# LikeLy-Journey/SegmenTron

Hardware: AMD Instinct MI355X
Metric: images/sec fwd+bwd DeepLabv3+_xception65 @1025x2049 (higher is better)
Workload: dtype bf16; 1 GPU; DeepLabv3+_xception65 train step (fwd + CE loss + bwd + SGD) @1025x2049, batch 2/GPU (BASELINE.json configs[2]); global_batch=2, bn=BN, parallelism=dp1, full_size=True

## Files before the change

segmentron_amd/csrc/optim.hip:

```cpp
#include "common.h"

namespace seg {

constexpr int SGD_TENSORS = 48;
constexpr int SGD_BLOCKS = 320;
constexpr int SGD_CHUNK = 16384;
constexpr int SGD_THREADS = 256;

struct SgdArgs {
  float* p[SGD_TENSORS];
  const float* g[SGD_TENSORS];
  float* m[SGD_TENSORS];
  int n[SGD_TENSORS];
  unsigned char group[SGD_TENSORS];
  unsigned char blk_tensor[SGD_BLOCKS];
  int blk_chunk[SGD_BLOCKS];
  const float* lr;
  const float* wd;
  float momentum;
  int first;
};

__global__ __launch_bounds__(SGD_THREADS) void sgd_multi_tensor_kernel(const SgdArgs a) {
  const int t = a.blk_tensor[blockIdx.x];
  const long base = (long)a.blk_chunk[blockIdx.x] * SGD_CHUNK;
  const int n = a.n[t];
  float* __restrict__ p = a.p[t];
  const float* __restrict__ g = a.g[t];
  float* __restrict__ m = a.m[t];
  const float lr = a.lr[a.group[t]], wd = a.wd[a.group[t]];
  const float mom = a.momentum;
  const bool vec = (n % 4) == 0;
  if (vec) {
    for (long i = base + threadIdx.x * 4; i < min((long)n, base + SGD_CHUNK); i += SGD_THREADS * 4) {
      float4 pv = *reinterpret_cast<float4*>(p + i);
      const float4 gv = *reinterpret_cast<const float4*>(g + i);
      float4 mv = make_float4(0.f, 0.f, 0.f, 0.f);
      if (!a.first) mv = *reinterpret_cast<float4*>(m + i);
      float pe[4] = {pv.x, pv.y, pv.z, pv.w}, me[4] = {mv.x, mv.y, mv.z, mv.w};
      const float ge[4] = {gv.x, gv.y, gv.z, gv.w};
#pragma unroll
      for (int k = 0; k < 4; ++k) {
        const float d = fmaf(wd, pe[k], ge[k]);
        me[k] = a.first ? d : fmaf(mom, me[k], d);
        pe[k] = fmaf(-lr, me[k], pe[k]);
      }
      *reinterpret_cast<float4*>(m + i) = make_float4(me[0], me[1], me[2], me[3]);
      *reinterpret_cast<float4*>(p + i) = make_float4(pe[0], pe[1], pe[2], pe[3]);
    }
  } else {
    for (long i = base + threadIdx.x; i < min((long)n, base + SGD_CHUNK); i += SGD_THREADS) {
      const float d = fmaf(wd, p[i], g[i]);
      const float mv = a.first ? d : fmaf(mom, m[i], d);
      m[i] = mv;
      p[i] = fmaf(-lr, mv, p[i]);
    }
  }
}

}

extern "C" int seg_sgd_multi_tensor(int ntensors, const void* const* params,
                                    const void* const* grads, const void* const* bufs,
                                    const long* numel, const int* group, const float* lr_dev,
                                    const float* wd_dev, float momentum, int first, void* stream) {
  using namespace seg;
  SEG_REQUIRE(ntensors >= 0 && lr_dev && wd_dev, "sgd_multi_tensor: bad arguments");
  SgdArgs a;
  a.lr = lr_dev; a.wd = wd_dev; a.momentum = momentum; a.first = first ? 1 : 0;
  int nt = 0, nb = 0;
  auto flush = [&]() -> int {
    if (nb == 0) { nt = 0; return 0; }
    hipLaunchKernelGGL(sgd_multi_tensor_kernel, dim3(nb), dim3(SGD_THREADS), 0,
                       (hipStream_t)stream, a);
    nt = nb = 0;
    return check_launch("sgd_multi_tensor");
  };
  for (int i = 0; i < ntensors; ++i) {
    SEG_REQUIRE(params[i] && grads[i] && bufs[i], "sgd_multi_tensor: null tensor %d", i);
    SEG_REQUIRE(numel[i] >= 0 && numel[i] < (1L << 31), "sgd_multi_tensor: tensor %d too large", i);
    SEG_REQUIRE(group[i] >= 0 && group[i] < 256, "sgd_multi_tensor: bad group %d", group[i]);
    const int chunks = (int)((numel[i] + SGD_CHUNK - 1) / SGD_CHUNK);
    int c = 0;
    while (c < chunks) {
      if (nt == SGD_TENSORS || nb == SGD_BLOCKS) {
        const int rc = flush();
        if (rc) return rc;
      }
      a.p[nt] = (float*)params[i]; a.g[nt] = (const float*)grads[i]; a.m[nt] = (float*)bufs[i];
      a.n[nt] = (int)numel[i]; a.group[nt] = (unsigned char)group[i];
      while (c < chunks && nb < SGD_BLOCKS) {
        a.blk_tensor[nb] = (unsigned char)nt;
        a.blk_chunk[nb] = c;
        ++nb; ++c;
      }
      ++nt;
    }
  }
  return flush();
}


namespace seg {

constexpr int PK_JOBS = 32, PK_BLOCKS = 480, PK_TILE = 64, PK_THREADS = 256;
constexpr int PK_SPAN = 4;

struct PackArgs {
  const float* src[PK_JOBS];
  void* dst[PK_JOBS];
  int O[PK_JOBS], C[PK_JOBS];
  unsigned char transpose[PK_JOBS];
  unsigned char blk_job[PK_BLOCKS];
  int blk_tile[PK_BLOCKS];
  int dtype;
};

template <typename T>
__global__ __launch_bounds__(PK_THREADS) void pack_multi_kernel(const PackArgs a) {
  __shared__ float tile[PK_TILE][PK_TILE + 1];
  const int j = a.blk_job[blockIdx.x];
  const int O = a.O[j], C = a.C[j];
  const int tc = (C + PK_TILE - 1) / PK_TILE, ntiles = ((O + PK_TILE - 1) / PK_TILE) * tc;
  const float* __restrict__ src = a.src[j];
  T* __restrict__ dst = reinterpret_cast<T*>(a.dst[j]);
  const int tx = threadIdx.x & 63, ty = threadIdx.x >> 6;
  const bool tr = a.transpose[j] != 0;
  for (int t = a.blk_tile[blockIdx.x]; t < min(ntiles, a.blk_tile[blockIdx.x] + PK_SPAN); ++t) {
    const int o0 = (t / tc) * PK_TILE, c0 = (t % tc) * PK_TILE;
    if (!tr) {
      for (int r = ty; r < PK_TILE; r += 4) {
        const int o = o0 + r, c = c0 + tx;
        if (o < O && c < C) Vec<T>::store1(dst + (long)o * C + c, src[(long)o * C + c]);
      }
      continue;
    }
    __syncthreads();
    for (int r = ty; r < PK_TILE; r += 4) {
      const int o = o0 + r, c = c0 + tx;
      tile[r][tx] = (o < O && c < C) ? src[(long)o * C + c] : 0.f;
    }
    __syncthreads();
    for (int r = ty; r < PK_TILE; r += 4) {
      const int c = c0 + r, o = o0 + tx;
      if (c < C && o < O) Vec<T>::store1(dst + (long)c * O + o, tile[tx][r]);
    }
  }
}

}

extern "C" int seg_pack_multi(int dtype, int njobs, const void* const* srcs, const void* const* dsts,
                              const int* O, const int* C, const int* transpose, void* stream) {
  using namespace seg;
  SEG_REQUIRE(dtype == DT_F32 || dtype == DT_BF16, "pack_multi: bad dtype %d", dtype);
  PackArgs a;
  a.dtype = dtype;
  int nj = 0, nb = 0;
  auto flush = [&]() -> int {
    if (nb == 0) { nj = 0; return 0; }
    if (dtype == DT_BF16)
      hipLaunchKernelGGL((pack_multi_kernel<bf16_t>), dim3(nb), dim3(PK_THREADS), 0,
                         (hipStream_t)stream, a);
    else
      hipLaunchKernelGGL((pack_multi_kernel<float>), dim3(nb), dim3(PK_THREADS), 0,
                         (hipStream_t)stream, a);
    nj = nb = 0;
    return check_launch("pack_multi");
  };
  for (int i = 0; i < njobs; ++i) {
    SEG_REQUIRE(srcs[i] && dsts[i] && O[i] >= 1 && C[i] >= 1, "pack_multi: bad job %d", i);
    const long to = (O[i] + PK_TILE - 1) / PK_TILE, tc = (C[i] + PK_TILE - 1) / PK_TILE;
    SEG_REQUIRE(to * tc < (1L << 30), "pack_multi: job %d too large", i);
    long t = 0;
    while (t < to * tc) {
      if (nj == PK_JOBS || nb == PK_BLOCKS) {
        const int rc = flush();
        if (rc) return rc;
      }
      a.src[nj] = (const float*)srcs[i]; a.dst[nj] = const_cast<void*>(dsts[i]);
      a.O[nj] = O[i]; a.C[nj] = C[i]; a.transpose[nj] = transpose[i] ? 1 : 0;
      while (t < to * tc && nb < PK_BLOCKS) {
        a.blk_job[nb] = (unsigned char)nj;
        a.blk_tile[nb] = (int)t;
        ++nb; t += PK_SPAN;
      }
      ++nj;
    }
  }
  return flush();
}
```

Baseline: 91.37 images/sec.

## Rework multi-tensor SGD and weight-pack kernels with binary-search block planning

Moves the SGD and pack launch planning into a shared header. Each block now finds its tensor by binary search over per-tensor first-block offsets, which lets one launch cover many more tensors and cuts launch count. SGD is templated on the first step, unrolled with nontemporal loads and stores, and uses smaller chunks. Pack merges a plain copy and a transposed copy of the same source into one job and uses vectorized 8-wide loads and stores. The costs are extra per-block search work and more complex alignment-dependent code paths.

```diff
diff --git a/segmentron_amd/csrc/optim.hip b/segmentron_amd/csrc/optim.hip
--- a/segmentron_amd/csrc/optim.hip
+++ b/segmentron_amd/csrc/optim.hip
@@ -1,57 +1,69 @@
 #include "common.h"
+#include "optim_plan.h"
 
 namespace seg {
 
-constexpr int SGD_TENSORS = 48;
-constexpr int SGD_BLOCKS = 320;
-constexpr int SGD_CHUNK = 16384;
-constexpr int SGD_THREADS = 256;
-
-struct SgdArgs {
-  float* p[SGD_TENSORS];
-  const float* g[SGD_TENSORS];
-  float* m[SGD_TENSORS];
-  int n[SGD_TENSORS];
-  unsigned char group[SGD_TENSORS];
-  unsigned char blk_tensor[SGD_BLOCKS];
-  int blk_chunk[SGD_BLOCKS];
-  const float* lr;
-  const float* wd;
-  float momentum;
-  int first;
-};
-
+__device__ __forceinline__ bool aligned16(const void* p) { return ((uintptr_t)p & 15) == 0; }
+
+__device__ __forceinline__ float4 ldg_nt(const float* p) {
+  const f32x4 v = __builtin_nontemporal_load(reinterpret_cast<const f32x4*>(p));
+  return make_float4(v.x, v.y, v.z, v.w);
+}
+__device__ __forceinline__ void stg_nt(float* p, const float4& v) {
+  const f32x4 t = {v.x, v.y, v.z, v.w};
+  __builtin_nontemporal_store(t, reinterpret_cast<f32x4*>(p));
+}
+
+template <bool FIRST>
 __global__ __launch_bounds__(SGD_THREADS) void sgd_multi_tensor_kernel(const SgdArgs a) {
-  const int t = a.blk_tensor[blockIdx.x];
-  const long base = (long)a.blk_chunk[blockIdx.x] * SGD_CHUNK;
+  const int t = plan_find(a.first_blk, a.nt, (int)blockIdx.x);
+  const long base = (long)((int)blockIdx.x - a.first_blk[t]) * SGD_CHUNK;
   const int n = a.n[t];
   float* __restrict__ p = a.p[t];
   const float* __restrict__ g = a.g[t];
   float* __restrict__ m = a.m[t];
   const float lr = a.lr[a.group[t]], wd = a.wd[a.group[t]];
   const float mom = a.momentum;
-  const bool vec = (n % 4) == 0;
+  const long end = min((long)n, base + SGD_CHUNK);
+  const bool vec = (n % 4) == 0 && aligned16(p) && aligned16(g) && aligned16(m);
   if (vec) {
-    for (long i = base + threadIdx.x * 4; i < min((long)n, base + SGD_CHUNK); i += SGD_THREADS * 4) {
-      float4 pv = *reinterpret_cast<float4*>(p + i);
-      const float4 gv = *reinterpret_cast<const float4*>(g + i);
-      float4 mv = make_float4(0.f, 0.f, 0.f, 0.f);
-      if (!a.first) mv = *reinterpret_cast<float4*>(m + i);
-      float pe[4] = {pv.x, pv.y, pv.z, pv.w}, me[4] = {mv.x, mv.y, mv.z, mv.w};
-      const float ge[4] = {gv.x, gv.y, gv.z, gv.w};
-#pragma unroll
-      for (int k = 0; k < 4; ++k) {
-        const float d = fmaf(wd, pe[k], ge[k]);
-        me[k] = a.first ? d : fmaf(mom, me[k], d);
-        pe[k] = fmaf(-lr, me[k], pe[k]);
-      }
-      *reinterpret_cast<float4*>(m + i) = make_float4(me[0], me[1], me[2], me[3]);
-      *reinterpret_cast<float4*>(p + i) = make_float4(pe[0], pe[1], pe[2], pe[3]);
+    for (long b = base; b < end; b += SGD_THREADS * 4 * SGD_UNROLL) {
+      long idx[SGD_UNROLL];
+      bool ok[SGD_UNROLL];
+      float4 pv[SGD_UNROLL], gv[SGD_UNROLL], mv[SGD_UNROLL];
+#pragma unroll
+      for (int u = 0; u < SGD_UNROLL; ++u) {
+        const long i = b + (long)(u * SGD_THREADS + (int)threadIdx.x) * 4;
+        ok[u] = i < end;
+        idx[u] = ok[u] ? i : end - 4;
+      }
+#pragma unroll
+      for (int u = 0; u < SGD_UNROLL; ++u) {
+        pv[u] = *reinterpret_cast<const float4*>(p + idx[u]);
+        gv[u] = ldg_nt(g + idx[u]);
+        mv[u] = FIRST ? make_float4(0.f, 0.f, 0.f, 0.f) : ldg_nt(m + idx[u]);
+      }
+#pragma unroll
+      for (int u = 0; u < SGD_UNROLL; ++u) {
+        float pe[4] = {pv[u].x, pv[u].y, pv[u].z, pv[u].w};
+        float me[4] = {mv[u].x, mv[u].y, mv[u].z, mv[u].w};
+        const float ge[4] = {gv[u].x, gv[u].y, gv[u].z, gv[u].w};
+#pragma unroll
+        for (int k = 0; k < 4; ++k) {
+          const float d = fmaf(wd, pe[k], ge[k]);
+          me[k] = FIRST ? d : fmaf(mom, me[k], d);
+          pe[k] = fmaf(-lr, me[k], pe[k]);
+        }
+        if (ok[u]) {
+          stg_nt(m + idx[u], make_float4(me[0], me[1], me[2], me[3]));
+          *reinterpret_cast<float4*>(p + idx[u]) = make_float4(pe[0], pe[1], pe[2], pe[3]);
+        }
+      }
     }
   } else {
-    for (long i = base + threadIdx.x; i < min((long)n, base + SGD_CHUNK); i += SGD_THREADS) {
+    for (long i = base + threadIdx.x; i < end; i += SGD_THREADS) {
       const float d = fmaf(wd, p[i], g[i]);
-      const float mv = a.first ? d : fmaf(mom, m[i], d);
+      const float mv = FIRST ? d : fmaf(mom, m[i], d);
       m[i] = mv;
       p[i] = fmaf(-lr, mv, p[i]);
     }
@@ -66,84 +78,106 @@
                                     const float* wd_dev, float momentum, int first, void* stream) {
   using namespace seg;
   SEG_REQUIRE(ntensors >= 0 && lr_dev && wd_dev, "sgd_multi_tensor: bad arguments");
+  for (int i = 0; i < ntensors; ++i) {
+    SEG_REQUIRE(numel[i] >= 0 && numel[i] < (1L << 31), "sgd_multi_tensor: tensor %d too large", i);
+    SEG_REQUIRE(numel[i] == 0 || (params[i] && grads[i] && bufs[i]),
+                "sgd_multi_tensor: null tensor %d", i);
+    SEG_REQUIRE(group[i] >= 0 && group[i] < 256, "sgd_multi_tensor: bad group %d", group[i]);
+  }
   SgdArgs a;
-  a.lr = lr_dev; a.wd = wd_dev; a.momentum = momentum; a.first = first ? 1 : 0;
-  int nt = 0, nb = 0;
-  auto flush = [&]() -> int {
-    if (nb == 0) { nt = 0; return 0; }
-    hipLaunchKernelGGL(sgd_multi_tensor_kernel, dim3(nb), dim3(SGD_THREADS), 0,
-                       (hipStream_t)stream, a);
-    nt = nb = 0;
+  a.lr = lr_dev; a.wd = wd_dev; a.momentum = momentum;
+  return sgd_plan(ntensors, params, grads, bufs, numel, group, a, [&](const SgdArgs& l, int nb) {
+    if (first)
+      hipLaunchKernelGGL(sgd_multi_tensor_kernel<true>, dim3(nb), dim3(SGD_THREADS), 0,
+                         (hipStream_t)stream, l);
+    else
+      hipLaunchKernelGGL(sgd_multi_tensor_kernel<false>, dim3(nb), dim3(SGD_THREADS), 0,
+                         (hipStream_t)stream, l);
     return check_launch("sgd_multi_tensor");
-  };
-  for (int i = 0; i < ntensors; ++i) {
-    SEG_REQUIRE(params[i] && grads[i] && bufs[i], "sgd_multi_tensor: null tensor %d", i);
-    SEG_REQUIRE(numel[i] >= 0 && numel[i] < (1L << 31), "sgd_multi_tensor: tensor %d too large", i);
-    SEG_REQUIRE(group[i] >= 0 && group[i] < 256, "sgd_multi_tensor: bad group %d", group[i]);
-    const int chunks = (int)((numel[i] + SGD_CHUNK - 1) / SGD_CHUNK);
-    int c = 0;
-    while (c < chunks) {
-      if (nt == SGD_TENSORS || nb == SGD_BLOCKS) {
-        const int rc = flush();
-        if (rc) return rc;
-      }
-      a.p[nt] = (float*)params[i]; a.g[nt] = (const float*)grads[i]; a.m[nt] = (float*)bufs[i];
-      a.n[nt] = (int)numel[i]; a.group[nt] = (unsigned char)group[i];
-      while (c < chunks && nb < SGD_BLOCKS) {
-        a.blk_tensor[nb] = (unsigned char)nt;
-        a.blk_chunk[nb] = c;
-        ++nb; ++c;
-      }
-      ++nt;
-    }
-  }
-  return flush();
+  });
 }
 
 
 namespace seg {
-
-constexpr int PK_JOBS = 32, PK_BLOCKS = 480, PK_TILE = 64, PK_THREADS = 256;
-constexpr int PK_SPAN = 4;
-
-struct PackArgs {
-  const float* src[PK_JOBS];
-  void* dst[PK_JOBS];
-  int O[PK_JOBS], C[PK_JOBS];
-  unsigned char transpose[PK_JOBS];
-  unsigned char blk_job[PK_BLOCKS];
-  int blk_tile[PK_BLOCKS];
-  int dtype;
-};
 
 template <typename T>
 __global__ __launch_bounds__(PK_THREADS) void pack_multi_kernel(const PackArgs a) {
+  constexpr int VEC = Vec<T>::N;
   __shared__ float tile[PK_TILE][PK_TILE + 1];
-  const int j = a.blk_job[blockIdx.x];
+  const int j = plan_find(a.first_blk, a.nj, (int)blockIdx.x);
+  const int t = (int)blockIdx.x - a.first_blk[j];
   const int O = a.O[j], C = a.C[j];
-  const int tc = (C + PK_TILE - 1) / PK_TILE, ntiles = ((O + PK_TILE - 1) / PK_TILE) * tc;
+  const int tc = (C + PK_TILE - 1) / PK_TILE;
+  const int o0 = (t / tc) * PK_TILE, c0 = (t % tc) * PK_TILE;
   const float* __restrict__ src = a.src[j];
   T* __restrict__ dst = reinterpret_cast<T*>(a.dst[j]);
-  const int tx = threadIdx.x & 63, ty = threadIdx.x >> 6;
-  const bool tr = a.transpose[j] != 0;
-  for (int t = a.blk_tile[blockIdx.x]; t < min(ntiles, a.blk_tile[blockIdx.x] + PK_SPAN); ++t) {
-    const int o0 = (t / tc) * PK_TILE, c0 = (t % tc) * PK_TILE;
-    if (!tr) {
-      for (int r = ty; r < PK_TILE; r += 4) {
-        const int o = o0 + r, c = c0 + tx;
-        if (o < O && c < C) Vec<T>::store1(dst + (long)o * C + c, src[(long)o * C + c]);
-      }
-      continue;
-    }
-    __syncthreads();
+  T* __restrict__ dst_t = reinterpret_cast<T*>(a.dst_t[j]);
+  const int tid = threadIdx.x;
+  if ((C % 8) == 0 && aligned16(src)) {
+    const int c8 = tid & 7, r = tid >> 3;
+    const int c = c0 + c8 * 8;
+    const bool cok = c < C;
+    const int cl = cok ? c : C - 8;
+    const bool wide_dst = dst != nullptr && aligned16(dst);
+    float4 w[2][2];
+#pragma unroll
+    for (int i = 0; i < 2; ++i) {
+      const int o = min(o0 + r + 32 * i, O - 1);
+      w[i][0] = *reinterpret_cast<const float4*>(src + (long)o * C + cl);
+      w[i][1] = *reinterpret_cast<const float4*>(src + (long)o * C + cl + 4);
+    }
+#pragma unroll
+    for (int i = 0; i < 2; ++i) {
+      const int ro = r + 32 * i, o = o0 + ro;
+      const float f[8] = {w[i][0].x, w[i][0].y, w[i][0].z, w[i][0].w,
+                          w[i][1].x, w[i][1].y, w[i][1].z, w[i][1].w};
+      if (dst != nullptr && o < O && cok) {
+        T* d = dst + (long)o * C + c;
+        if (wide_dst) {
+#pragma unroll
+          for (int k = 0; k < 8; k += VEC) Vec<T>::store(d + k, f + k);
+        } else {
+#pragma unroll
+          for (int k = 0; k < 8; ++k) Vec<T>::store1(d + k, f[k]);
+        }
+      }
+      if (dst_t != nullptr) {
+#pragma unroll
+        for (int k = 0; k < 8; ++k) tile[ro][c8 * 8 + k] = f[k];
+      }
+    }
+  } else {
+    const int tx = tid & 63, ty = tid >> 6;
     for (int r = ty; r < PK_TILE; r += 4) {
       const int o = o0 + r, c = c0 + tx;
-      tile[r][tx] = (o < O && c < C) ? src[(long)o * C + c] : 0.f;
-    }
-    __syncthreads();
+      const bool ok = o < O && c < C;
+      const float v = ok ? src[(long)o * C + c] : 0.f;
+      if (ok && dst != nullptr) Vec<T>::store1(dst + (long)o * C + c, v);
+      if (dst_t != nullptr) tile[r][tx] = v;
+    }
+  }
+  if (dst_t == nullptr) return;
+  __syncthreads();
+  if ((O % 8) == 0 && aligned16(dst_t)) {
+#pragma unroll
+    for (int i = 0; i < 2; ++i) {
+      const int idx = tid + PK_THREADS * i;
+      const int og = idx & 7, cl = idx >> 3;
+      const int o = o0 + og * 8, c = c0 + cl;
+      if (c < C && o < O) {
+        float f[8];
+#pragma unroll
+        for (int k = 0; k < 8; ++k) f[k] = tile[og * 8 + k][cl];
+        T* d = dst_t + (long)c * O + o;
+#pragma unroll
+        for (int k = 0; k < 8; k += VEC) Vec<T>::store(d + k, f + k);
+      }
+    }
+  } else {
+    const int tx = tid & 63, ty = tid >> 6;
     for (int r = ty; r < PK_TILE; r += 4) {
       const int c = c0 + r, o = o0 + tx;
-      if (c < C && o < O) Vec<T>::store1(dst + (long)c * O + o, tile[tx][r]);
+      if (c < C && o < O) Vec<T>::store1(dst_t + (long)c * O + o, tile[tx][r]);
     }
   }
 }
@@ -154,39 +188,18 @@
                               const int* O, const int* C, const int* transpose, void* stream) {
   using namespace seg;
   SEG_REQUIRE(dtype == DT_F32 || dtype == DT_BF16, "pack_multi: bad dtype %d", dtype);
+  for (int i = 0; i < njobs; ++i) {
+    SEG_REQUIRE(srcs[i] && dsts[i] && O[i] >= 1 && C[i] >= 1, "pack_multi: bad job %d", i);
+    SEG_REQUIRE(pack_tiles(O[i], C[i]) < (1L << 30), "pack_multi: job %d too large", i);
+  }
   PackArgs a;
-  a.dtype = dtype;
-  int nj = 0, nb = 0;
-  auto flush = [&]() -> int {
-    if (nb == 0) { nj = 0; return 0; }
+  return pack_plan(njobs, srcs, dsts, O, C, transpose, a, [&](const PackArgs& l, int nb) {
     if (dtype == DT_BF16)
       hipLaunchKernelGGL((pack_multi_kernel<bf16_t>), dim3(nb), dim3(PK_THREADS), 0,
-                         (hipStream_t)stream, a);
+                         (hipStream_t)stream, l);
     else
       hipLaunchKernelGGL((pack_multi_kernel<float>), dim3(nb), dim3(PK_THREADS), 0,
-                         (hipStream_t)stream, a);
-    nj = nb = 0;
+                         (hipStream_t)stream, l);
     return check_launch("pack_multi");
-  };
-  for (int i = 0; i < njobs; ++i) {
-    SEG_REQUIRE(srcs[i] && dsts[i] && O[i] >= 1 && C[i] >= 1, "pack_multi: bad job %d", i);
-    const long to = (O[i] + PK_TILE - 1) / PK_TILE, tc = (C[i] + PK_TILE - 1) / PK_TILE;
-    SEG_REQUIRE(to * tc < (1L << 30), "pack_multi: job %d too large", i);
-    long t = 0;
-    while (t < to * tc) {
-      if (nj == PK_JOBS || nb == PK_BLOCKS) {
-        const int rc = flush();
-        if (rc) return rc;
-      }
-      a.src[nj] = (const float*)srcs[i]; a.dst[nj] = const_cast<void*>(dsts[i]);
-      a.O[nj] = O[i]; a.C[nj] = C[i]; a.transpose[nj] = transpose[i] ? 1 : 0;
-      while (t < to * tc && nb < PK_BLOCKS) {
-        a.blk_job[nb] = (unsigned char)nj;
-        a.blk_tile[nb] = (int)t;
-        ++nb; t += PK_SPAN;
-      }
-      ++nj;
-    }
-  }
-  return flush();
-}
+  });
+}
diff --git a/segmentron_amd/csrc/optim_plan.h b/segmentron_amd/csrc/optim_plan.h
--- /dev/null
+++ b/segmentron_amd/csrc/optim_plan.h
@@ -0,0 +1,125 @@
+#pragma once
+#include <stdint.h>
+#include <vector>
+
+#if defined(__HIPCC__)
+#define SEG_PLAN_HD __host__ __device__ __forceinline__
+#else
+#define SEG_PLAN_HD inline
+#endif
+
+namespace seg {
+
+constexpr int PLAN_ARG_BYTES = 4096;
+
+SEG_PLAN_HD int plan_find(const int* first, int n, int blk) {
+  int lo = 0, hi = n;
+  while (hi - lo > 1) {
+    const int mid = (lo + hi) >> 1;
+    if (first[mid] <= blk) lo = mid; else hi = mid;
+  }
+  return lo;
+}
+
+constexpr int SGD_TENSORS = 110;
+constexpr int SGD_THREADS = 256;
+constexpr int SGD_UNROLL = 2;
+constexpr int SGD_CHUNK = 2048;
+
+struct SgdArgs {
+  float* p[SGD_TENSORS];
+  const float* g[SGD_TENSORS];
+  float* m[SGD_TENSORS];
+  int n[SGD_TENSORS];
+  int first_blk[SGD_TENSORS];
+  unsigned char group[SGD_TENSORS];
+  const float* lr;
+  const float* wd;
+  float momentum;
+  int nt;
+};
+static_assert(sizeof(SgdArgs) <= PLAN_ARG_BYTES, "SgdArgs must fit the kernel argument block");
+static_assert(SGD_CHUNK % (SGD_THREADS * 4 * SGD_UNROLL) == 0, "whole trips per chunk");
+
+template <class Launch>
+int sgd_plan(int ntensors, const void* const* params, const void* const* grads,
+             const void* const* bufs, const long* numel, const int* group, SgdArgs& a,
+             Launch&& launch) {
+  int nt = 0, nb = 0;
+  for (int i = 0; i < ntensors; ++i) {
+    if (numel[i] == 0) continue;
+    if (nt == SGD_TENSORS) {
+      a.nt = nt;
+      const int rc = launch(a, nb);
+      if (rc) return rc;
+      nt = nb = 0;
+    }
+    a.p[nt] = (float*)params[i]; a.g[nt] = (const float*)grads[i]; a.m[nt] = (float*)bufs[i];
+    a.n[nt] = (int)numel[i]; a.group[nt] = (unsigned char)group[i];
+    a.first_blk[nt] = nb;
+    nb += (int)((numel[i] + SGD_CHUNK - 1) / SGD_CHUNK);
+    ++nt;
+  }
+  if (nt == 0) return 0;
+  a.nt = nt;
+  return launch(a, nb);
+}
+
+constexpr int PK_JOBS = 100;
+constexpr int PK_TILE = 64, PK_THREADS = 256;
+constexpr long PK_MAX_BLOCKS = 1L << 30;
+
+struct PackArgs {
+  const float* src[PK_JOBS];
+  void* dst[PK_JOBS];
+  void* dst_t[PK_JOBS];
+  int O[PK_JOBS], C[PK_JOBS];
+  int first_blk[PK_JOBS];
+  int nj;
+};
+static_assert(sizeof(PackArgs) <= PLAN_ARG_BYTES, "PackArgs must fit the kernel argument block");
+
+inline long pack_tiles(int O, int C) {
+  return (long)((O + PK_TILE - 1) / PK_TILE) * ((C + PK_TILE - 1) / PK_TILE);
+}
+
+template <class Launch>
+int pack_plan(int njobs, const void* const* srcs, const void* const* dsts, const int* O,
+              const int* C, const int* transpose, PackArgs& a, Launch&& launch) {
+  int nj = 0;
+  long nb = 0;
+  std::vector<unsigned char> taken(njobs > 0 ? njobs : 0, 0);
+  for (int i = 0; i < njobs; ++i) {
+    if (taken[i]) continue;
+    int partner = -1;
+    for (int k = i + 1; k < njobs; ++k) {
+      if (!taken[k] && srcs[k] == srcs[i] && O[k] == O[i] && C[k] == C[i] &&
+          (transpose[k] != 0) != (transpose[i] != 0)) {
+        partner = k;
+        break;
+      }
+    }
+    const long tiles = pack_tiles(O[i], C[i]);
+    if (nj == PK_JOBS || nb + tiles > PK_MAX_BLOCKS) {
+      a.nj = nj;
+      const int rc = launch(a, (int)nb);
+      if (rc) return rc;
+      nj = 0; nb = 0;
+    }
+    a.src[nj] = (const float*)srcs[i]; a.O[nj] = O[i]; a.C[nj] = C[i];
+    a.dst[nj] = a.dst_t[nj] = nullptr;
+    (transpose[i] ? a.dst_t[nj] : a.dst[nj]) = const_cast<void*>(dsts[i]);
+    if (partner >= 0) {
+      (transpose[partner] ? a.dst_t[nj] : a.dst[nj]) = const_cast<void*>(dsts[partner]);
+      taken[partner] = 1;
+    }
+    a.first_blk[nj] = (int)nb;
+    nb += tiles;
+    ++nj;
+  }
+  if (nj == 0) return 0;
+  a.nj = nj;
+  return launch(a, (int)nb);
+}
+
+}
```

After: 92.15 images/sec, median of 6. No clear change (+0.8%).
